# maua-maua-maua/maua

Measured on AMD Instinct MI355X. Metric: frames/sec (whole node), 1024x1024 StyleGAN2 audio-reactive render, higher is better.
Workload: dtype bf16

## Files before the change

### maua_amd/csrc/internal.h

```cpp
#pragma once
#include "common.h"

namespace maua {

int launch_pack_rgb8(hipStream_t stream, const float* img, uint8_t* out, int B, int H, int W);
template <typename TI, typename TO>
int launch_nchw_to_nhwc(hipStream_t s, const void* x, void* y, int N, int C, int HW, int Cp);
template <typename TI, typename TO>
int launch_nhwc_to_nchw(hipStream_t s, const void* x, void* y, int N, int C, int HW, int Cp);

struct ConvArgs {
  const void* x;
  long x_bstride;
  const void* w;
  const float* s;
  const float* d;
  const float* noise;
  long noise_bstride;
  float noise_strength;
  const float* noise_scale;
  const float* bias;
  void* y;
  int B, H, W, Ci, Co, up;
  int act;
// ... 60 lines not shown
  const float* noise;
  long noise_bstride;
  float noise_strength;
  const float* noise_scale;
  const float* bias;
  void* y;
  int B, H, W, Ci, Co, up, act;
  float alpha, gain, clamp;
  const float* rgb_wmod;
  const float* rgb_bias;
  const float* rgb_prev;
  float* rgb_out;
  float rgb_clamp;
  float fir[16];
  uint8_t* rgb8_out;
  int rgb_skip_f32;
};
bool hires_supported(int dtype, int Ci, int Co, int up, int H, int W);
int launch_modconv_hires(hipStream_t stream, const HiresArgs& a, int dtype = MAUA_BF16);
bool upwalk_supported(int dtype, int Ci, int Co, int up, int H, int W);
size_t upwalk_weight_elems(int Co, int Ci);
int launch_upwalk(hipStream_t stream, const HiresArgs& a, int dtype = MAUA_BF16);
int launch_prep_upwalk_weights(hipStream_t stream, const float* w, void* wt, int Co, int Ci, int flip, int dtype = MAUA_BF16);
bool upwalk_fused_supported(int dtype, int Ci, int Cm, int H, int W);
int launch_upwalk_fused(hipStream_t stream, const HiresArgs& up, const HiresArgs& c1, int force_segs = 0, int narrow_ok = 1,
                        int dtype = MAUA_BF16);

int launch_prep_weights(hipStream_t stream, int dtype, const float* w, void* wt, float* wsq, int Co, int Ci, int k,
                        int up, int flip, int Cop, int Cip);
int launch_f32_split_inplace(hipStream_t stream, void* w, long n_floats);

int launch_tconv2(hipStream_t stream, int dtype, const ConvArgs& a);
bool tconv_dma_supported(int dtype, int Ci, int Co, int H, int W);
int launch_tconv_dma(hipStream_t stream, const ConvArgs& a, int dtype = MAUA_BF16);
int launch_tconv_edges(hipStream_t stream, const ConvArgs& a, int dtype = MAUA_BF16);
int launch_prep_tconv_weights(hipStream_t stream, int dtype, const float* w, void* wt, int Co, int Ci, int flip);

struct UpfirArgs {
  const void* t;
  void* y;
  const float* d;
  const float* noise;
  long noise_bstride;
  float noise_strength;
  const float* noise_scale;
  const float* bias;
  const float* out_scale;
  int B, H, W, Co;
  int act;
  float alpha, gain, clamp;
};
int launch_upfir_epilogue(hipStream_t stream, int dtype, const UpfirArgs& a);
bool tconv_fir_supported(int dtype, int Ci, int Co, int H, int W);
int launch_tconv_fir(hipStream_t stream, const ConvArgs& a, const UpfirArgs& u, int dtype = MAUA_BF16);
size_t prepped_weight_elems(int k, int up, int Cop, int Cip);

struct LayerOperands { const void* x; const void* w; const float* s; const float* d; const float* bias; void* y; int B, H, W, Ci, Co, up; };
struct NoiseOperands { const float* noise; long bstride; float strength; const float* scale; };
struct Epilogue { int act; float alpha, gain, clamp; };
template <typename A>
inline void set_noise_args(A& a, const NoiseOperands& n) {
  a.noise = n.noise; a.noise_bstride = n.bstride; a.noise_strength = n.strength; a.noise_scale = n.scale;
}
template <typename A>
inline void set_epilogue_args(A& a, const Epilogue& e) {
  a.act = e.act; a.alpha = e.alpha; a.gain = e.gain; a.clamp = e.clamp;
}
template <typename A>
inline A layer_args(A a, const LayerOperands& l, const NoiseOperands& n, const Epilogue& e) {
  a.x = l.x; a.w = l.w; a.s = l.s; a.d = l.d; a.bias = l.bias; a.y = l.y;
  a.B = l.B; a.H = l.H; a.W = l.W; a.Ci = l.Ci; a.Co = l.Co; a.up = l.up;
  set_noise_args(a, n);
  set_epilogue_args(a, e);
  return a;
}
template <typename A>
inline void fuse_torgb_args(A& a, const float* wmod, const float* bias, const float* prev, float* out, float clamp, const float* fir16) {
  a.rgb_wmod = wmod; a.rgb_bias = bias; a.rgb_prev = prev; a.rgb_out = out; a.rgb_clamp = clamp;
  for (int i = 0; i < 16; i++) a.fir[i] = fir16[i];
}
inline void pack_u8_args(HiresArgs& a, uint8_t* rgb8_out, bool skip_f32) {
  a.rgb8_out = rgb8_out;
  a.rgb_skip_f32 = skip_f32;
}
inline ConvArgs tconv_args(const void* x, long x_bstride, const void* w, const float* s, void* t, int B, int H, int W, int Ci, int Co) {
  ConvArgs a{};
  a.x = x; a.x_bstride = x_bstride; a.w = w; a.s = s; a.y = t;
  a.B = B; a.H = H; a.W = W; a.Ci = Ci; a.Co = Co; a.up = 2;
  return a;
}
inline UpfirArgs upfir_args(void* y, const float* d, const float* bias, const float* out_scale, int B, int H, int W, int Co,
                            const NoiseOperands& n, const Epilogue& e) {
  UpfirArgs u{};
  u.y = y; u.d = d; u.bias = bias; u.out_scale = out_scale; u.B = B; u.H = H; u.W = W; u.Co = Co;
  set_noise_args(u, n);
  set_epilogue_args(u, e);
  return u;
}
inline void upsample_fir16(float* fir) {
  const float g4[4] = {0.25f, 0.75f, 0.75f, 0.25f};
  for (int u = 0; u < 4; u++)
    for (int v = 0; v < 4; v++) fir[u * 4 + v] = g4[u] * g4[v];
}

int modconv3x3_check(int dtype, const ConvArgs& a);
int lowres_check(int dtype, const ConvArgs& a);
int lowres_ksplit(int dtype, int B, int H, int W, int Ci, int Co, int up);
// ... 213 lines not shown
```

### maua_amd/csrc/modconv_api.hip

```cpp
#include <algorithm>
#include <cstring>

#include "common.h"
#include "internal.h"

namespace maua {
namespace {

enum { R_LOWRES = 0, R_GENERIC, R_DMA, R_HIRES, R_UPWALK, R_FUSED, R_WALKDONE, R_TFIR, R_TDMA, R_T2, R_UPFIR };

bool is_tconv(int r) { return r == R_TFIR || r == R_TDMA || r == R_T2; }
bool reads_premod(int r) { return r == R_TFIR || r == R_TDMA || r == R_DMA; }

LayerOperands operands(const maua_modconv_desc* d) {
  return LayerOperands{d->x, nullptr, d->s, d->d, d->bias, d->y, d->B, d->H, d->W, d->Ci, d->Co, d->up};
}
NoiseOperands noise_of(const maua_modconv_desc* d) { return NoiseOperands{d->noise, d->noise_bstride, d->noise_strength, d->noise_scale}; }
Epilogue epilogue_of(const maua_modconv_desc* d) { return Epilogue{d->act, d->alpha, d->gain, d->clamp}; }

template <typename A>
A desc_args(const maua_modconv_desc* d) {
  A a = layer_args(A{}, operands(d), noise_of(d), epilogue_of(d));
  if (d->rgb_out) {
    float fir[16];
// ... 140 lines not shown
  if (route == R_UPWALK || route == R_FUSED) {
    if (int rc = launch_prep_upwalk_weights(st, d->w, base + o_w, d->Co, d->Ci, d->flip, dtype)) return rc;
  } else if (is_tconv(route)) {
    if (int rc = launch_prep_tconv_weights(st, dtype, d->w, base + o_w, d->Co, d->Ci, d->flip)) return rc;
  } else if (route != R_UPFIR) {
    if (int rc = launch_prep_weights(st, dtype, d->w, base + o_w, nullptr, d->Co, d->Ci, 3, d->up, d->up == 2 ? d->flip : 0, d->Co, d->Ci))
      return rc;
  }
  if (route == R_FUSED)
    if (int rc = launch_prep_weights(st, dtype, d1->w, base + o_w1, nullptr, d1->Co, d1->Ci, 3, 1, 0, d1->Co, d1->Ci)) return rc;
  const void* x = d->x;
  long x_bstride = d->x_bstride;
  if (reads_premod(route)) {
    if (int rc = launch_premod_nhwc(st, d->x, d->x_bstride, d->s, base + o_xm, d->B, (long)d->H * d->W, d->Ci, dtype)) return rc;
    x = base + o_xm;
    x_bstride = (long)d->H * d->W * d->Ci;
  }
  if (ones_bytes) {
    const long n = (long)d->B * d->Ci;
    hipLaunchKernelGGL(modconv_fill_ones_kernel, dim3((unsigned)((n + 255) / 256)), dim3(256), 0, st, (float*)(base + o_ones), n);
    MAUA_HIP_CHECK(hipGetLastError());
  }
  switch (route) {
    case R_LOWRES:
    case R_GENERIC:
    case R_DMA: {
      ConvArgs a = conv_args(d);
      a.x = x; a.x_bstride = x_bstride; a.w = base + o_w;
      if (route == R_DMA) a.s = nullptr;
      return route == R_LOWRES    ? launch_modconv_lowres(st, dtype, a, base + o_xm, (float*)(base + o_ws))
             : route == R_GENERIC ? launch_modconv3x3(st, dtype, a)
                                  : launch_modconv_dma(st, a, dtype);
    }
    case R_HIRES:
    case R_UPWALK:
    case R_FUSED: {
      HiresArgs a = hires_args(d);
      a.w = base + o_w;
      if (route == R_HIRES) return launch_modconv_hires(st, a, dtype);
      if (route == R_UPWALK) return launch_upwalk(st, a, dtype);
      HiresArgs f = hires_args(d1);
      f.x = nullptr; f.y = nullptr; f.w = base + o_w1;
      a.y = nullptr;
      return launch_upwalk_fused(st, a, f, force_segs, narrow_ok, dtype);
    }
    case R_TFIR:
    case R_TDMA:
    case R_T2: {
      void* t = d->t ? d->t : base + o_t;
      ConvArgs a = tconv_args(d);
      a.x = x; a.x_bstride = x_bstride; a.w = base + o_w; a.y = t;
      if (route != R_T2) a.s = (const float*)(base + o_ones);
      UpfirArgs u = upfir_args(d);
      if (route == R_TFIR) return launch_tconv_fir(st, a, u, dtype);
      if (route == R_TDMA) {
        if (int rc = launch_tconv_edges(st, a, dtype)) return rc;
        if (int rc = launch_tconv_dma(st, a, dtype)) return rc;
      } else if (int rc = launch_tconv2(st, dtype, a)) {
        return rc;
      }
      u.t = t;
      return launch_upfir_epilogue(st, dtype, u);
    }
    case R_UPFIR: {
      UpfirArgs u = upfir_args(d);
      u.t = d->x;
      return launch_upfir_epilogue(st, dtype, u);
    }
  }
  return MAUA_OK;
}

extern "C" int maua_torgb_ex(maua_ctx* ctx, const void* x, const float* wmod, const float* bias, const float* prev, float* out, int B,
                             int H, int W, int C, float clamp, int dtype) {
  MAUA_REQUIRE(ctx && x && wmod && bias && out, "maua_torgb_ex: NULL argument");
  MAUA_REQUIRE(B >= 0 && H > 0 && W > 0 && C > 0, "maua_torgb_ex: bad shape");
  MAUA_REQUIRE(!prev || (H % 2 == 0 && W % 2 == 0), "maua_torgb_ex: the skip image needs an even grid");
  RgbArgs r{};
  r.x = x; r.wmod = wmod; r.bias = bias; r.prev = prev; r.out = out; r.B = B; r.H = H; r.W = W; r.C = C; r.clamp = clamp;
  upsample_fir16(r.fir);
  return launch_torgb(ctx->stream, dtype, r);
}
```

### maua_amd/csrc/modconv_tconv_fir.hip

```cpp
#include "common.h"
#include "internal.h"

namespace maua {

namespace {

constexpr int PTW = 32;
constexpr int HW1 = PTW + 1;
constexpr int KB = 64;
constexpr int WROWS = 9 * 32;
constexpr int WBUF = WROWS * KB;
constexpr int OFF_H = 2 * WBUF;
constexpr int ES = 128 * 2;

__device__ __constant__ const int kSlotF[9] = {0, 1, 1, 2, 2, 3, 3, 3, 3};
__device__ __constant__ const int kClsF[9] = {0, 0, 1, 0, 2, 0, 1, 2, 3};

__device__ __forceinline__ unsigned lds_off(const void* p) {
  return (unsigned)(size_t)(__attribute__((address_space(3))) const void*)p;
}
__device__ __forceinline__ void dma16_s(const void* sbase, unsigned voff, unsigned lds_dst) {
  asm volatile("s_mov_b32 m0, %2\n\ts_nop 0\n\tglobal_load_lds_dwordx4 %0, %1" ::"v"(voff), "s"(sbase), "s"(lds_dst)
               : "memory");
}
template <typename F>
__device__ __forceinline__ void mma(f32x16& acc, const u32x4& w, const u32x4& x) {
  Mma16<F>::step(acc, w, x);
}
__device__ __forceinline__ int swz(int n) { return (n >> 2) & 3; }

__device__ __forceinline__ int t_col(int tc, int pc) {
  const int p = tc >> 1;
  return p * ES + ((((tc & 1) ^ (p & 3)) << 6) | ((pc ^ ((p >> 2) & 3)) << 4));
}

template <typename F>
__device__ __forceinline__ void fir_hrow(const char* tile, int tr, const int (&tcol)[5], f32x2_t (&h)[2][4]) {
  f32x2_t c[5][4];
  const int rowb = (tr >> 1) * (PTW * ES), rsw = (tr & 1) << 7;
#pragma unroll
  for (int rx = 0; rx < 5; rx++) {
    const u32x4 v = *reinterpret_cast<const u32x4*>(tile + rowb + (tcol[rx] ^ rsw));
#pragma unroll
    for (int k = 0; k < 4; k++) c[rx][k] = f32x2_t{Fmt16<F>::lo(v[k]), Fmt16<F>::hi(v[k])};
  }
#pragma unroll
  for (int e = 0; e < 4; e++) {
    h[0][e] = (c[0][e] + c[3][e]) + 3.f * (c[1][e] + c[2][e]);
    h[1][e] = (c[1][e] + c[4][e]) + 3.f * (c[2][e] + c[3][e]);
  }
}

}

template <int PTH_, typename F>
__global__ __launch_bounds__(PTH_ * 32, PTH_ == 8 ? 2 : 1) void tconv_fir_kernel(ConvArgs a, UpfirArgs u) {
  constexpr int PTH = PTH_, UPR = PTH - 2;
  constexpr int HPX = (PTH + 1) * HW1, HBUF = HPX * KB;
  constexpr int NW = PTH / 2, NT = NW * 64;
  constexpr int WJ = (WBUF / 1024 + NW - 1) / NW, HJ = (HPX * 4 + NT - 1) / NT;
  constexpr int FG = NT / 128, FROWS = 2 * UPR / FG;
  static_assert(FG * FROWS == 2 * UPR, "output rows must split evenly over the FIR groups");
  extern __shared__ __attribute__((aligned(1024))) char smem[];
  const unsigned lds0 = __builtin_amdgcn_readfirstlane(lds_off(smem));
  const int tid = threadIdx.x, lane = tid & 63;
  const int wave = __builtin_amdgcn_readfirstlane(tid >> 6);
  const int r = lane & 31, h = lane >> 5;
  const int tiles_x = (a.W + 29) / 30, tiles = tiles_x * ((a.H + UPR - 1) / UPR), CB = a.Co >> 5;
  const int cbg = CB < 8 ? CB : 8, n_ts = tiles * a.B, per_group = ((n_ts + 7) >> 3) * 8 * cbg;
  const int L = blockIdx.x, grp = L / per_group, Lg = L - grp * per_group;
  const int xcd = Lg & 7, idx = Lg >> 3;
  const int cb = grp * cbg + idx % cbg, ts = (idx / cbg) * 8 + xcd;
  if (ts >= n_ts) return;
  const int b = ts / tiles, tile = ts - b * tiles;
  const int tyi = tile / tiles_x, txi = tile - tyi * tiles_x;
  const int ty0 = tyi * UPR - 1, tx0 = txi * 30 - 1;
  const char* xb = reinterpret_cast<const char*>(a.x) + (long)b * a.x_bstride * 2;
  const char* wp = reinterpret_cast<const char*>(a.w);

  unsigned hoff[HJ];
#pragma unroll
  for (int j = 0; j < HJ; j++) {
    const int P = (wave + NW * j) * 64 + lane;
    const int hp = P >> 2, q = (P & 3) ^ swz(hp);
    const int py = (hp * 1986) >> 16;
    const int px = hp - py * HW1;
    const int gy = ty0 - 1 + py, gx = tx0 - 1 + px;
    hoff[j] = 0xffffffffu;
    if (P < HPX * 4) {
      if (gy >= 0 && gx >= 0 && gy < a.H && gx < a.W) {
        hoff[j] = (unsigned)(((gy * a.W + gx) * a.Ci + q * 8) * 2);
      } else {
        *reinterpret_cast<u32x4*>(smem + OFF_H + P * 16) = u32x4{0u, 0u, 0u, 0u};
        *reinterpret_cast<u32x4*>(smem + OFF_H + HBUF + P * 16) = u32x4{0u, 0u, 0u, 0u};
      }
    }
  }
  unsigned woff[WJ];
#pragma unroll
  for (int j = 0; j < WJ; j++) {
    const int ii = wave + NW * j;
    const int R = min(16 * ii + (lane >> 2), WROWS - 1);
    const int k = R >> 5, n = R & 31;
    const int q = (lane & 3) ^ swz(R);
    woff[j] = (unsigned)((((((kSlotF[k] * CB + cb) * 4 + kClsF[k]) * 32 + n) * a.Ci) + q * 8) * 2);
  }
#define TD_ISSUE(C_, BUF_)                                                                               \
  {                                                                                                      \
    const char* ws_ = wp + (long)(C_) * KB;                                                              \
    _Pragma("unroll") for (int j = 0; j < WJ; j++)                                                      \
      if (wave + NW * j < WBUF / 1024) dma16_s(ws_, woff[j], lds0 + (BUF_) * WBUF + (wave + NW * j) * 1024); \
    const char* xs_ = xb + (long)(C_) * KB;                                                              \
    _Pragma("unroll") for (int j = 0; j < HJ; j++)                                                      \
      if (hoff[j] != 0xffffffffu) dma16_s(xs_, hoff[j], lds0 + OFF_H + (BUF_) * HBUF + (wave + NW * j) * 1024); \
  }

  const int hp00 = (2 * wave) * HW1 + r;
  const unsigned b0 = (unsigned)(r * KB + ((swz(r) ^ h) << 4));
#define TD_A(HR_, Q1_, KS_, BUF_)                                                                        \
  ({                                                                                                     \
    const int hp_ = hpv + (HR_) * HW1 + (Q1_);                                                           \
    *reinterpret_cast<const u32x4*>(smem + ((OFF_H + (BUF_) * HBUF + hp_ * KB + ((swz(hp_) ^ h) << 4)) ^ ((KS_) << 5))); \
  })
#define TD_B(K_, KS_, BUF_) (*reinterpret_cast<const u32x4*>(smem + (BUF_) * WBUF + (K_) * 32 * KB + (b0 ^ ((KS_) << 5))))

  f32x16 acc[2][4];
#pragma unroll
  for (int R = 0; R < 2; R++)
#pragma unroll
    for (int c = 0; c < 4; c++)
#pragma unroll
      for (int e = 0; e < 16; e++) acc[R][c][e] = 0.f;

  const int n_chunks = a.Ci >> 5;
  TD_ISSUE(0, 0)
  if (n_chunks > 1) TD_ISSUE(1, 1)
  asm volatile("s_waitcnt vmcnt(0)" ::: "memory");
  __syncthreads();
  int hpv = hp00;
#define TD_STEP(KS_, BUF_)                                                                               \
  {                                                                                                      \
    u32x4 A00 = TD_A(0, 0, KS_, BUF_), A01 = TD_A(0, 1, KS_, BUF_);      \
    u32x4 A10 = TD_A(1, 0, KS_, BUF_), A11 = TD_A(1, 1, KS_, BUF_);                    \
    u32x4 A20 = TD_A(2, 0, KS_, BUF_), A21 = TD_A(2, 1, KS_, BUF_);                    \
    {                                                                                                    \
      const u32x4 B0 = TD_B(0, KS_, BUF_), B1 = TD_B(1, KS_, BUF_), B2 = TD_B(2, KS_, BUF_);              \
      mma<F>(acc[0][0], B0, A00); mma<F>(acc[1][0], B0, A10);                                 \
      mma<F>(acc[0][1], B2, A01); mma<F>(acc[1][1], B2, A11);                        \
      mma<F>(acc[0][0], B1, A01); mma<F>(acc[1][0], B1, A11);                        \
    }                                                                                                    \
    {                                                                                                    \
      const u32x4 B3 = TD_B(3, KS_, BUF_), B4 = TD_B(4, KS_, BUF_);                                       \
      mma<F>(acc[0][2], B4, A10); mma<F>(acc[1][2], B4, A20);                        \
      mma<F>(acc[0][0], B3, A10); mma<F>(acc[1][0], B3, A20);                        \
    }                                                                                                    \
    {                                                                                                    \
      const u32x4 B5 = TD_B(5, KS_, BUF_), B6 = TD_B(6, KS_, BUF_), B7 = TD_B(7, KS_, BUF_), B8 = TD_B(8, KS_, BUF_); \
      mma<F>(acc[0][3], B8, A11); mma<F>(acc[1][3], B8, A21);                                 \
      mma<F>(acc[0][1], B6, A11); mma<F>(acc[1][1], B6, A21);                                                  \
      mma<F>(acc[0][2], B7, A11); mma<F>(acc[1][2], B7, A21);                                                  \
      mma<F>(acc[0][0], B5, A11); mma<F>(acc[1][0], B5, A21);                                                  \
    }                                                                                                    \
  }
  for (int c = 0; c < n_chunks; c++) {
    const int buf = c & 1;
    asm volatile("" : "+v"(hpv));
    TD_STEP(0, buf)
    {
      u32x4 A00 = TD_A(0, 0, 1, buf), A01 = TD_A(0, 1, 1, buf), A10 = TD_A(1, 0, 1, buf), A11 = TD_A(1, 1, 1, buf);
      u32x4 A20 = TD_A(2, 0, 1, buf), A21 = TD_A(2, 1, 1, buf);
      const u32x4 B0 = TD_B(0, 1, buf), B1 = TD_B(1, 1, buf), B2 = TD_B(2, 1, buf), B3 = TD_B(3, 1, buf), B4 = TD_B(4, 1, buf);
      const u32x4 B5 = TD_B(5, 1, buf), B6 = TD_B(6, 1, buf), B7 = TD_B(7, 1, buf), B8 = TD_B(8, 1, buf);
      asm volatile("s_waitcnt vmcnt(0)" ::: "memory");
      __syncthreads();
      if (c + 2 < n_chunks) TD_ISSUE(c + 2, buf)
      mma<F>(acc[0][0], B0, A00); mma<F>(acc[1][0], B0, A10);
      mma<F>(acc[0][1], B2, A01); mma<F>(acc[1][1], B2, A11);
      mma<F>(acc[0][0], B1, A01); mma<F>(acc[1][0], B1, A11);
      mma<F>(acc[0][2], B4, A10); mma<F>(acc[1][2], B4, A20);
      mma<F>(acc[0][0], B3, A10); mma<F>(acc[1][0], B3, A20);
      mma<F>(acc[0][3], B8, A11); mma<F>(acc[1][3], B8, A21);
      mma<F>(acc[0][1], B6, A11); mma<F>(acc[1][1], B6, A21);
      mma<F>(acc[0][2], B7, A11); mma<F>(acc[1][2], B7, A21);
      mma<F>(acc[0][0], B5, A11); mma<F>(acc[1][0], B5, A21);
    }
  }
#undef TD_ISSUE
#undef TD_A
#undef TD_B
#undef TD_STEP

  const int fhalf = tid / 120, fw = tid - fhalf * 120;
  const int strip = fw >> 2, pc = fw & 3;
  const int xl = 2 + 2 * strip, yl0 = 2 + FROWS * fhalf;
  const int X = 2 * tx0 + xl, Wo = 2 * a.W, Ho = 2 * a.H;
  const int cho = cb * 32 + pc * 8;
  const bool fir_on = tid < 120 * FG && X < Wo;
  f32x2_t dv[4], bv[4], sv[4];
  float2 nzv[FROWS];
#pragma unroll
  for (int k = 0; k < FROWS; k++) nzv[k] = make_float2(0.f, 0.f);
  if (fir_on) {
#pragma unroll
    for (int e4 = 0; e4 < 8; e4 += 4) {
      const float4 s4 = u.out_scale ? *reinterpret_cast<const float4*>(u.out_scale + (long)b * a.Co + cho + e4)
                                    : make_float4(1.f, 1.f, 1.f, 1.f);
      sv[e4 / 2] = f32x2_t{s4.x, s4.y}; sv[e4 / 2 + 1] = f32x2_t{s4.z, s4.w};
      const float4 d4 = u.d ? *reinterpret_cast<const float4*>(u.d + (long)b * a.Co + cho + e4) : make_float4(1.f, 1.f, 1.f, 1.f);
      const float4 b4 = u.bias ? *reinterpret_cast<const float4*>(u.bias + cho + e4) : make_float4(0.f, 0.f, 0.f, 0.f);
      dv[e4 / 2] = f32x2_t{d4.x, d4.y}; dv[e4 / 2 + 1] = f32x2_t{d4.z, d4.w};
      bv[e4 / 2] = f32x2_t{b4.x, b4.y}; bv[e4 / 2 + 1] = f32x2_t{b4.z, b4.w};
    }
    if (u.noise) {
      const float* nb = u.noise + (long)b * u.noise_bstride;
#pragma unroll
      for (int k = 0; k < FROWS; k++) {
        const int Y = 2 * ty0 + yl0 + k;
        if (Y < Ho) nzv[k] = *reinterpret_cast<const float2*>(nb + (long)Y * Wo + X);
      }
    }
  }
  __syncthreads();
  char* tt = smem;
#pragma unroll
  for (int R = 0; R < 2; R++) {
    const int m = (2 * wave + R) * 32 + r;
#pragma unroll
    for (int c = 0; c < 4; c++)
#pragma unroll
      for (int qd = 0; qd < 4; qd++)
        *reinterpret_cast<uint2*>(tt + m * ES + (((c ^ (r & 3)) << 6) | ((qd ^ ((r >> 2) & 3)) << 4) | (h << 3))) =
            make_uint2(Fmt16<F>::pack2(acc[R][c][qd * 4 + 0], acc[R][c][qd * 4 + 1]), Fmt16<F>::pack2(acc[R][c][qd * 4 + 2], acc[R][c][qd * 4 + 3]));
  }
  __syncthreads();
  {
    if (fir_on) {
#pragma unroll
      for (int e = 0; e < 4; e++) { dv[e] *= 0.0625f * u.gain; bv[e] *= u.gain; }
      const float nzs = u.noise_strength * u.gain * (u.noise_scale ? u.noise_scale[b] : 1.f);
      const float cl = u.clamp >= 0.f ? u.clamp : 3.0e38f;
      char* yb = reinterpret_cast<char*>(u.y) + (long)b * Ho * Wo * a.Co * 2;
      int tcol[5];
#pragma unroll
      for (int rx = 0; rx < 5; rx++) tcol[rx] = t_col(xl - 1 + rx, pc);
      f32x2_t hr[4][2][4];
      fir_hrow<F>(tt, yl0 - 1, tcol, hr[0]);
      fir_hrow<F>(tt, yl0, tcol, hr[1]);
      fir_hrow<F>(tt, yl0 + 1, tcol, hr[2]);
#pragma unroll
      for (int k = 0; k < FROWS; k++) {
        fir_hrow<F>(tt, yl0 + k + 2, tcol, hr[(k + 3) & 3]);
        const int Y = 2 * ty0 + yl0 + k;
        if (Y < Ho) {
          const float nz[2] = {nzv[k].x * nzs, nzv[k].y * nzs};
#pragma unroll
          for (int j = 0; j < 2; j++) {
            f32x2_t o[4];
#pragma unroll
            for (int e = 0; e < 4; e++) {
              const f32x2_t accv = (hr[k & 3][j][e] + hr[(k + 3) & 3][j][e]) + 3.f * (hr[(k + 1) & 3][j][e] + hr[(k + 2) & 3][j][e]);
              f32x2_t t = accv * dv[e] + (bv[e] + nz[j]);
              const f32x2_t ta = t * u.alpha;
              t = f32x2_t{fmaxf(t[0], ta[0]), fmaxf(t[1], ta[1])};
              o[e] = f32x2_t{__builtin_amdgcn_fmed3f(t[0], -cl, cl), __builtin_amdgcn_fmed3f(t[1], -cl, cl)} * sv[e];
            }
            *reinterpret_cast<u32x4*>(yb + (((long)Y * Wo + X + j) * a.Co + cho) * 2) =
                u32x4{Fmt16<F>::pack2(o[0][0], o[0][1]), Fmt16<F>::pack2(o[1][0], o[1][1]), Fmt16<F>::pack2(o[2][0], o[2][1]), Fmt16<F>::pack2(o[3][0], o[3][1])};
          }
        }
      }
    }
  }
}

bool tconv_fir_supported(int dtype, int Ci, int Co, int H, int W) {
  return (dtype == MAUA_BF16 || dtype == MAUA_F16) && Ci % 32 == 0 && Co % 32 == 0 && H >= 16 && W >= 32 && (long)H * W * Ci * 2 < (1L << 32) &&
         16L * Co * Ci * 2 < (1L << 32);
}

int tconv_fir_check(const ConvArgs& a, const UpfirArgs& u, int dtype) {
  MAUA_REQUIRE(tconv_fir_supported(dtype, a.Ci, a.Co, a.H, a.W), "tconv_fir: unsupported shape");
  MAUA_REQUIRE(u.act == MAUA_ACT_LRELU && u.alpha >= 0.f && u.alpha <= 1.f && u.gain > 0.f, "tconv_fir: lrelu epilogue only");
  MAUA_REQUIRE(!u.noise || (((uintptr_t)u.noise % 8) == 0 && u.noise_bstride % 2 == 0), "tconv_fir: noise must be 8-byte aligned");
  const int pth = 8, upr = pth - 2;
  const int tiles = ((a.H + upr - 1) / upr) * ((a.W + 29) / 30), CB = a.Co / 32, cbg = CB < 8 ? CB : 8;
  MAUA_REQUIRE(CB % cbg == 0, "tconv_fir: channel blocks must split into groups of 8");
  const long n_ts = (long)tiles * a.B, grid = ((n_ts + 7) / 8) * 8 * cbg * (CB / cbg);
  MAUA_REQUIRE(grid < (1L << 31), "tconv_fir: grid too large");
  return MAUA_OK;
}

int launch_tconv_fir(hipStream_t stream, const ConvArgs& a, const UpfirArgs& u, int dtype) {
  if (int rc = tconv_fir_check(a, u, dtype)) return rc;
  if (a.B == 0) return MAUA_OK;
  const int pth = 8, upr = pth - 2;
  const int tiles = ((a.H + upr - 1) / upr) * ((a.W + 29) / 30), CB = a.Co / 32, cbg = CB < 8 ? CB : 8;
  const long n_ts = (long)tiles * a.B, grid = ((n_ts + 7) / 8) * 8 * cbg * (CB / cbg);
  const size_t smem = std::max<size_t>((size_t)2 * WBUF + 2 * (pth + 1) * HW1 * KB, (size_t)pth * PTW * ES);
  if (dtype == MAUA_F16) {
    MAUA_HIP_CHECK(hipFuncSetAttribute((const void*)tconv_fir_kernel<8, f16_t>, hipFuncAttributeMaxDynamicSharedMemorySize, (int)smem));
    hipLaunchKernelGGL((tconv_fir_kernel<8, f16_t>), dim3((unsigned)grid), dim3(256), smem, stream, a, u);
  } else {
    MAUA_HIP_CHECK(hipFuncSetAttribute((const void*)tconv_fir_kernel<8, bf16_t>, hipFuncAttributeMaxDynamicSharedMemorySize, (int)smem));
    hipLaunchKernelGGL((tconv_fir_kernel<8, bf16_t>), dim3((unsigned)grid), dim3(256), smem, stream, a, u);
  }
  MAUA_HIP_CHECK(hipGetLastError());
  return MAUA_OK;
}

}
```

### maua_amd/csrc/synth.hip

```cpp
#include <cmath>
#include <cstring>
#include <string>
#include <vector>

#include "common.h"
#include "internal.h"

using namespace maua;

namespace {

struct ConvLayer {
  int block, which;
  int Ci, Co, res, up, w_index;
  int ih = 0, iw = 0;
  int oh = 0, ow = 0;
  int fh = 0, fw = 0;
  float* affine_w = nullptr;
  float* affine_b = nullptr;
  float* bias = nullptr;
  float* noise_const = nullptr;
  float noise_strength = 0.f;
  void* wt = nullptr;
  void* wt_t = nullptr;
  void* wt_h = nullptr;
  float* wsq = nullptr;
  float* s = nullptr;
  float* d = nullptr;
  void* feat = nullptr;
};
struct RgbLayer {
  int block, C, res, w_index;
  int h = 0, w = 0;
  float* affine_w = nullptr;
  float* affine_b = nullptr;
  float* wrgb = nullptr;
  float* bias = nullptr;
  float* s = nullptr;
  float* wmod = nullptr;
};

template <typename T>
int dev_alloc(T** p, size_t n) {
  MAUA_HIP_CHECK(hipMalloc((void**)p, n * sizeof(T)));
  return MAUA_OK;
}

}

struct maua_synth {
  maua_ctx* ctx;
  int res, w_dim, channel_base, channel_max, dtype, nv_compat;
  int nblocks, num_ws;
  size_t esize;
  std::vector<ConvLayer> convs;
  std::vector<RgbLayer> rgbs;
  void* const_x = nullptr;
  int keep_features = 0;
  int lowres = 1;
  int use_hires = 1;
  int upwalk = 2;
  int walk_segs = 0;
  int walk_narrow = 1;
  int fuse_torgb = 1;
  int tconv_up = 1;
  int tconv_fir = 256;
  const float* nz_scales = nullptr;
  long nz_scale_stride = 0;
  int dma_conv = 1;
  int dual_store = 1;
  int tconv_dma = 1;
  float* ones = nullptr;
  void* xm = nullptr;
  void* tbuf = nullptr;
  void* lowres_xm = nullptr;
  float* lowres_ws = nullptr;
  int rs_layer = -1, rs_mode = 0, rs_th = 0, rs_tw = 0, rs_pl = 0, rs_pr = 0, rs_pt = 0, rs_pb = 0, rs_how = 3;
  float rs_value = 0.f;
  float* rs_noise = nullptr;
  void* const_rs = nullptr;
  float* rgb_tmp[2] = {nullptr, nullptr};
  int out_h = 0, out_w = 0;
  int warp_layer[3] = {-1, -1, -1};
  const float* warp_minv[3] = {nullptr, nullptr, nullptr};
  int profile = 0;
  std::vector<hipEvent_t> ev;
  size_t ev_used = 0;
  std::vector<size_t> ev_fwd_start;
  int bcap = 0;
  void* act[2] = {nullptr, nullptr};
  float* img[2] = {nullptr, nullptr};
  StyleLayer* style_table_dev = nullptr;
  float fir[16];
};

static void prof_mark(maua_synth* n) {
  if (!n->profile || n->ev_used >= (1u << 16)) return;
  if (n->ev_used == n->ev.size()) {
    hipEvent_t e;
    if (hipEventCreate(&e) != hipSuccess) return;
    n->ev.push_back(e);
  }
  hipEventRecord(n->ev[n->ev_used++], n->ctx->stream);
}

static int channels_for(int res, int base, int maxc) { return std::min(base / res, maxc); }

static bool lowres_fits(const maua_synth* n, const ConvLayer& c) {
  return lowres_supported(n->dtype, c.Ci, c.Co, c.up, c.ih, c.iw);
}
static bool tconv_dma_fits(const maua_synth* n, const ConvLayer& c) {
  return c.up == 2 && tconv_dma_supported(n->dtype, c.Ci, c.Co, c.ih, c.iw);
}

static void compute_dims(maua_synth* n) {
  int h = 4, w = 4;
  if (n->rs_layer == 0) { h = n->rs_th; w = n->rs_tw; }
  size_t li = 0;
  for (int blk = 0; blk < n->nblocks; blk++) {
// ... 362 lines not shown
    MAUA_HIP_CHECK(hipMemcpy(n->rs_noise, fill_noise_host, cnt * sizeof(float), hipMemcpyHostToDevice));
  }
  compute_dims(n);
  free_workspace(n);
  for (size_t i = 0; i < n->convs.size(); i++) {
    ConvLayer& c = n->convs[i];
    if (c.oh != before[i].oh || c.ow != before[i].ow) {
      hipFree(c.noise_const);
      c.noise_const = nullptr;
      MAUA_HIP_CHECK(hipMalloc((void**)&c.noise_const, (size_t)c.oh * c.ow * sizeof(float)));
      MAUA_HIP_CHECK(hipMemset(c.noise_const, 0, (size_t)c.oh * c.ow * sizeof(float)));
    }
  }
  return MAUA_OK;
}

int maua_synth_set_warp(maua_synth* n, int slot, int layer, const float* inv_matrices_dev) {
  MAUA_REQUIRE(n, "maua_synth_set_warp: net is NULL");
  MAUA_REQUIRE(slot >= 0 && slot < 3, "maua_synth_set_warp: slot must be 0..2");
  MAUA_REQUIRE(layer >= 1 && layer <= (int)n->convs.size(), "maua_synth_set_warp: layer must name a synthesis layer (1-based index into layer_names)");
  n->warp_layer[slot] = inv_matrices_dev ? layer : -1;
  n->warp_minv[slot] = inv_matrices_dev;
  return MAUA_OK;
}

int maua_synth_layer_size(const maua_synth* n, int layer, int* h, int* w) {
  MAUA_REQUIRE(n && h && w, "maua_synth_layer_size: NULL argument");
  MAUA_REQUIRE(layer >= -1 && layer < (int)n->convs.size(), "maua_synth_layer_size: no such layer");
  if (layer < 0) { *h = n->out_h; *w = n->out_w; }
  else { *h = n->convs[layer].oh; *w = n->convs[layer].ow; }
  return MAUA_OK;
}

int maua_synth_set_option(maua_synth* n, const char* key, int value) {
  MAUA_REQUIRE(n && key, "maua_synth_set_option: NULL argument");
  if (!strcmp(key, "profile")) {
    n->profile = value;
    n->ev_used = 0;
    n->ev_fwd_start.clear();
    return MAUA_OK;
  }
  if (!strcmp(key, "keep_features")) {
    if (n->keep_features != value) {
      MAUA_HIP_CHECK(hipStreamSynchronize(n->ctx->stream));
      free_workspace(n);
      n->keep_features = value;
    }
    return MAUA_OK;
  }
  static const std::pair<const char*, int maua_synth::*> routing[] = {
      {"lowres", &maua_synth::lowres},         {"use_hires", &maua_synth::use_hires}, {"upwalk", &maua_synth::upwalk},
      {"walk_segs", &maua_synth::walk_segs},   {"walk_narrow", &maua_synth::walk_narrow},
      {"fuse_torgb", &maua_synth::fuse_torgb}, {"tconv_up", &maua_synth::tconv_up},   {"tconv_fir", &maua_synth::tconv_fir},
      {"tconv_dma", &maua_synth::tconv_dma},   {"dma_conv", &maua_synth::dma_conv},   {"dual_store", &maua_synth::dual_store}};
  for (const auto& o : routing)
    if (!strcmp(key, o.first)) {
      n->*o.second = value;
      return MAUA_OK;
    }
  return fail(std::string("maua_synth_set_option: unknown option ") + key);
}

static thread_local hipMemcpyKind g_load_kind = hipMemcpyHostToDevice;

static int upload(float* dst, const float* host, size_t count, size_t expect, const char* name) {
  if (count != expect)
    return fail(std::string("maua_synth_load: ") + name + ": expected " + std::to_string(expect) + " values, got " +
                std::to_string(count));
  MAUA_HIP_CHECK(hipMemcpy(dst, host, count * sizeof(float), g_load_kind));
  return MAUA_OK;
}

int maua_synth_load(maua_synth* n, const char* name, const float* host, size_t count) {
  MAUA_REQUIRE(n && name && host, "maua_synth_load: NULL argument");
  std::string s(name);
  int blk = -1, pos = 0;
  if (sscanf(name, "bs.%d.%n", &blk, &pos) < 1 || blk < 0 || blk >= n->nblocks || pos == 0)
    return fail("maua_synth_load: unknown parameter name: " + s);
  std::string rest = s.substr(pos);
  hipStream_t st = n->ctx->stream;
  auto check_filter = [&]() -> int {
    if (count != 16) return fail("maua_synth_load: " + s + ": only the 4x4 [1,3,3,1] resample filter is supported");
    const float t[4] = {1, 3, 3, 1};
    for (int u = 0; u < 4; u++)
      for (int v = 0; v < 4; v++)
        if (std::fabs(host[u * 4 + v] - t[u] * t[v] / 64.f) > 1e-6f)
          return fail("maua_synth_load: " + s + ": only the 4x4 [1,3,3,1] resample filter is supported");
    return MAUA_OK;
  };
  if (rest == "resample_filter") return check_filter();
  if (rest == "const") {
    if (blk != 0) return fail("maua_synth_load: only block 0 has a const input");
    int C = n->convs[0].Ci;
    if (count != (size_t)C * 16) return fail("maua_synth_load: bs.0.const: wrong size");
    float* tmp;
    MAUA_HIP_CHECK(hipMalloc((void**)&tmp, count * 4));
    MAUA_HIP_CHECK(hipMemcpy(tmp, host, count * 4, g_load_kind));
    int rc = n->dtype == MAUA_BF16   ? launch_nchw_to_nhwc<float, bf16_t>(st, tmp, n->const_x, 1, C, 16, C)
             : n->dtype == MAUA_F16 ? launch_nchw_to_nhwc<float, f16_t>(st, tmp, n->const_x, 1, C, 16, C)
                                    : launch_nchw_to_nhwc<float, float>(st, tmp, n->const_x, 1, C, 16, C);
    hipStreamSynchronize(st);
    hipFree(tmp);
    return rc;
  }
  size_t dot = rest.find('.');
  if (dot == std::string::npos) return fail("maua_synth_load: unknown parameter name: " + s);
// ... 115 lines not shown
      const ConvLayer& c = n->convs[li];
      const Step& s = plan.conv[li];
      const bool hooked = n->rs_layer == (int)li + 1;
      void* y = n->keep_features && !hooked ? c.feat : n->act[cur];
      const float* next_s = s.scale_next ? n->convs[li + 1].s : nullptr;
      switch (s.route) {
        case Route::Lowres:
        case Route::Generic:
        case Route::DmaConv1: {
          ConvArgs a = layer_args(ConvArgs{}, li, x, y);
          a.x_bstride = x_bstride;
          a.out_scale = next_s;
          if (s.dual) a.y_scaled = n->xm;
          if (s.rgb) fuse_torgb(a);
          if (s.route == Route::DmaConv1) a.s = nullptr;
          if (int rc = s.route == Route::Lowres    ? launch_modconv_lowres(st, n->dtype, a, n->lowres_xm, n->lowres_ws)
                       : s.route == Route::Generic ? launch_modconv3x3(st, n->dtype, a)
                                                   : launch_modconv_dma(st, a, n->dtype))
            return rc;
          break;
        }
        case Route::Hires:
        case Route::Upwalk:
        case Route::FusedWalk: {
          HiresArgs a = layer_args(HiresArgs{}, li, x, s.skip_store ? nullptr : y);
          if (s.rgb) fuse_torgb(a);
          if (s.rgb8) pack_u8(a);
          if (s.route != Route::Hires) a.w = c.wt_h;
          if (s.route != Route::FusedWalk) {
            if (int rc = s.route == Route::Hires ? launch_modconv_hires(st, a, n->dtype) : launch_upwalk(st, a, n->dtype)) return rc;
            break;
          }
          HiresArgs f = layer_args(HiresArgs{}, li + 1, nullptr, nullptr);
          fuse_torgb(f);
          if (plan.conv[li + 1].rgb8) pack_u8(f);
          if (int rc = launch_upwalk_fused(st, a, f, n->walk_segs, n->walk_narrow, n->dtype)) return rc;
          break;
        }
        case Route::WalkDone:
          break;
        case Route::TconvFir:
        case Route::TconvDma:
        case Route::Tconv2: {
          ConvArgs a = tconv_args(x, x_bstride, c.wt_t, c.s, n->tbuf, B, c.ih, c.iw, c.Ci, c.Co);
          UpfirArgs u = upfir_args(y, c.d, c.bias, next_s, B, c.ih, c.iw, c.Co, layer_noise(li), lrelu_epilogue());
          if (s.src == Src::PremodPass)
            if (int rc = launch_premod_nhwc(st, x, x_bstride, c.s, n->xm, B, (long)c.ih * c.iw, c.Ci, n->dtype)) return rc;
          if (s.src == Src::PremodPass || s.src == Src::Xm) {
            a.x = n->xm;
            a.x_bstride = (long)c.ih * c.iw * c.Ci;
          }
          if (reads_premod(s.route)) a.s = n->ones;
          if (s.route == Route::TconvFir) {
            if (int rc = launch_tconv_fir(st, a, u, n->dtype)) return rc;
            prof_mark(n);
            break;
          }
          if (s.route == Route::TconvDma) {
            if (int rc = launch_tconv_edges(st, a, n->dtype)) return rc;
            if (int rc = launch_tconv_dma(st, a, n->dtype)) return rc;
          } else if (int rc = launch_tconv2(st, n->dtype, a)) {
            return rc;
          }
          prof_mark(n);
          u.t = n->tbuf;
          if (int rc = launch_upfir_epilogue(st, n->dtype, u)) return rc;
          break;
        }
      }
      prof_mark(n);
      x = y;
      x_bstride = (long)c.oh * c.ow * c.Co;
      cur ^= 1;
      if (hooked) {
        void* dst = n->keep_features ? c.feat : n->act[cur];
        if (int rc = resize_feat(x, x_bstride, B, c.oh, c.ow, c.Co, dst)) return rc;
        x = dst;
        x_bstride = (long)c.fh * c.fw * c.Co;
        cur ^= 1;
      }
      for (int wsl = 0; wsl < 3; wsl++) {
        if (n->warp_layer[wsl] != (int)li + 1 || !n->warp_minv[wsl]) continue;
        void* dst = n->act[cur];
        if (dst == x) dst = n->act[cur ^ 1];
        if (int rc = launch_warp_affine_nhwc(st, n->dtype, x, dst, n->warp_minv[wsl], B, c.fh, c.fw, c.Co)) return rc;
        if (n->keep_features) {
          MAUA_HIP_CHECK(hipMemcpyAsync(c.feat, dst, (size_t)B * c.fh * c.fw * c.Co * n->esize, hipMemcpyDeviceToDevice, st));
        } else {
          x = dst;
          cur = (dst == n->act[0]) ? 1 : 0;
        }
      }
    }
    if (plan.rgb[blk] != RgbRoute::Fused) {
      const bool hook = plan.rgb[blk] == RgbRoute::Hook;
      RgbArgs r{};
      r.x = x; r.wmod = g.wmod; r.bias = g.bias; r.prev = hook ? nullptr : prev_img;
      r.out = hook ? n->rgb_tmp[0] : rgb_out; r.B = B; r.H = g.h; r.W = g.w; r.C = g.C; r.clamp = 256.f;
      memcpy(r.fir, n->fir, sizeof(r.fir));
      if (int rc = launch_torgb(st, n->dtype, r)) return rc;
      if (hook) {
        const ConvLayer& hc = n->convs[n->rs_layer - 1];
        const int nh = hc.oh, nw = hc.ow;
        ResizeArgs inv{};
        inv.x = n->rgb_tmp[0]; inv.x_bstride = 3L * g.h * g.w; inv.y = n->rgb_tmp[1]; inv.B = B; inv.H = g.h; inv.W = g.w;
        inv.C = 3; inv.oh = nh; inv.ow = nw; inv.mode = n->rs_mode; inv.pl = -n->rs_pl; inv.pt = -n->rs_pt;
        inv.how = MAUA_PAD_CONSTANT; inv.value = 0.f; inv.noise = nullptr;
// ... 91 lines not shown
```

Measured before the change: 4589.

## Walk tconv+FIR tiles vertically, carrying halo t rows between steps

Adds a walking variant of the fused transposed-conv + FIR kernel. Each block now steps down a column segment in 8-row steps and carries the last three t rows in registers/LDS, so the overlapping halo rows are no longer recomputed as they are with independent 6-row tiles. A host-side planner chooses the segment count from the CU count to balance occupancy against walk length, and the mode is on by default. The cost is longer-running blocks with a sequential dependency, extra LDS, and fewer blocks available for parallelism.

```diff
diff --git a/maua_amd/csrc/internal.h b/maua_amd/csrc/internal.h
--- a/maua_amd/csrc/internal.h
+++ b/maua_amd/csrc/internal.h
@@ -136,7 +136,7 @@
 };
 int launch_upfir_epilogue(hipStream_t stream, int dtype, const UpfirArgs& a);
 bool tconv_fir_supported(int dtype, int Ci, int Co, int H, int W);
-int launch_tconv_fir(hipStream_t stream, const ConvArgs& a, const UpfirArgs& u, int dtype = MAUA_BF16);
+int launch_tconv_fir(hipStream_t stream, const ConvArgs& a, const UpfirArgs& u, int dtype = MAUA_BF16, int walk = 1, int force_segs = 0);
 size_t prepped_weight_elems(int k, int up, int Cop, int Cip);
 
 struct LayerOperands { const void* x; const void* w; const float* s; const float* d; const float* bias; void* y; int B, H, W, Ci, Co, up; };
diff --git a/maua_amd/csrc/modconv_api.hip b/maua_amd/csrc/modconv_api.hip
--- a/maua_amd/csrc/modconv_api.hip
+++ b/maua_amd/csrc/modconv_api.hip
@@ -216,7 +216,7 @@
       a.x = x; a.x_bstride = x_bstride; a.w = base + o_w; a.y = t;
       if (route != R_T2) a.s = (const float*)(base + o_ones);
       UpfirArgs u = upfir_args(d);
-      if (route == R_TFIR) return launch_tconv_fir(st, a, u, dtype);
+      if (route == R_TFIR) return launch_tconv_fir(st, a, u, dtype, force_segs >= 0, force_segs);
       if (route == R_TDMA) {
         if (int rc = launch_tconv_edges(st, a, dtype)) return rc;
         if (int rc = launch_tconv_dma(st, a, dtype)) return rc;
diff --git a/maua_amd/csrc/modconv_tconv_fir.hip b/maua_amd/csrc/modconv_tconv_fir.hip
--- a/maua_amd/csrc/modconv_tconv_fir.hip
+++ b/maua_amd/csrc/modconv_tconv_fir.hip
@@ -53,20 +53,22 @@
 
 }
 
-template <int PTH_, typename F>
-__global__ __launch_bounds__(PTH_ * 32, PTH_ == 8 ? 2 : 1) void tconv_fir_kernel(ConvArgs a, UpfirArgs u) {
+template <int PTH_, typename F, bool WALK>
+__global__ __launch_bounds__(PTH_ * 32, PTH_ == 8 ? 2 : 1) void tconv_fir_kernel(ConvArgs a, UpfirArgs u, int nseg, int seg_steps) {
   constexpr int PTH = PTH_, UPR = PTH - 2;
+  static_assert(!WALK || PTH_ == 8, "the walk carries three t rows of a 16-row tile");
   constexpr int HPX = (PTH + 1) * HW1, HBUF = HPX * KB;
   constexpr int NW = PTH / 2, NT = NW * 64;
   constexpr int WJ = (WBUF / 1024 + NW - 1) / NW, HJ = (HPX * 4 + NT - 1) / NT;
-  constexpr int FG = NT / 128, FROWS = 2 * UPR / FG;
-  static_assert(FG * FROWS == 2 * UPR, "output rows must split evenly over the FIR groups");
+  constexpr int FG = NT / 128, FROWS = (WALK ? 2 * PTH : 2 * UPR) / FG;
+  static_assert(FG * FROWS == (WALK ? 2 * PTH : 2 * UPR), "output rows must split evenly over the FIR groups");
+  constexpr int OFF_T = WALK ? 2 * PTW * ES : 0;
   extern __shared__ __attribute__((aligned(1024))) char smem[];
   const unsigned lds0 = __builtin_amdgcn_readfirstlane(lds_off(smem));
   const int tid = threadIdx.x, lane = tid & 63;
   const int wave = __builtin_amdgcn_readfirstlane(tid >> 6);
   const int r = lane & 31, h = lane >> 5;
-  const int tiles_x = (a.W + 29) / 30, tiles = tiles_x * ((a.H + UPR - 1) / UPR), CB = a.Co >> 5;
+  const int tiles_x = (a.W + 29) / 30, tiles = tiles_x * (WALK ? nseg : (a.H + UPR - 1) / UPR), CB = a.Co >> 5;
   const int cbg = CB < 8 ? CB : 8, n_ts = tiles * a.B, per_group = ((n_ts + 7) >> 3) * 8 * cbg;
   const int L = blockIdx.x, grp = L / per_group, Lg = L - grp * per_group;
   const int xcd = Lg & 7, idx = Lg >> 3;
@@ -74,14 +76,56 @@
   if (ts >= n_ts) return;
   const int b = ts / tiles, tile = ts - b * tiles;
   const int tyi = tile / tiles_x, txi = tile - tyi * tiles_x;
-  const int ty0 = tyi * UPR - 1, tx0 = txi * 30 - 1;
+  const int tx0 = txi * 30 - 1;
+  int step = 0, step_end = 1, y_lo = 0, y_hi = 2 * a.H;
+  if (WALK) {
+    const int n_steps = (a.H >> 3) + 1, s0 = tyi ? seg_steps + (tyi - 1) * (seg_steps - 1) : 0;
+    step_end = min(n_steps, tyi ? s0 + seg_steps - 1 : seg_steps);
+    step = tyi ? s0 - 1 : 0;
+    y_lo = tyi ? 16 * s0 - 2 : 0;
+    if (step_end < n_steps) y_hi = 16 * step_end - 2;
+  }
   const char* xb = reinterpret_cast<const char*>(a.x) + (long)b * a.x_bstride * 2;
   const char* wp = reinterpret_cast<const char*>(a.w);
 
+  unsigned woff[WJ];
+#pragma unroll
+  for (int j = 0; j < WJ; j++) {
+    const int ii = wave + NW * j;
+    const int R = min(16 * ii + (lane >> 2), WROWS - 1);
+    const int k = R >> 5, n = R & 31;
+    const int q = (lane & 3) ^ swz(R);
+    woff[j] = (unsigned)((((((kSlotF[k] * CB + cb) * 4 + kClsF[k]) * 32 + n) * a.Ci) + q * 8) * 2);
+  }
+#define TD_ISSUE(C_, BUF_)                                                                               \
+  {                                                                                                      \
+    const char* ws_ = wp + (long)(C_) * KB;                                                              \
+    _Pragma("unroll") for (int j = 0; j < WJ; j++)                                                      \
+      if (wave + NW * j < WBUF / 1024) dma16_s(ws_, woff[j], lds0 + (BUF_) * WBUF + (wave + NW * j) * 1024); \
+    const char* xs_ = xb + (long)(C_) * KB;                                                              \
+    _Pragma("unroll") for (int j = 0; j < HJ; j++)                                                      \
+      if (hoff[j] != 0xffffffffu) dma16_s(xs_, hoff[j], lds0 + OFF_H + (BUF_) * HBUF + (wave + NW * j) * 1024); \
+  }
+
+  const int hp00 = (2 * wave) * HW1 + r;
+  const unsigned b0 = (unsigned)(r * KB + ((swz(r) ^ h) << 4));
+#define TD_A(HR_, Q1_, KS_, BUF_)                                                                        \
+  ({                                                                                                     \
+    const int hp_ = hpv + (HR_) * HW1 + (Q1_);                                                           \
+    *reinterpret_cast<const u32x4*>(smem + ((OFF_H + (BUF_) * HBUF + hp_ * KB + ((swz(hp_) ^ h) << 4)) ^ ((KS_) << 5))); \
+  })
+#define TD_B(K_, KS_, BUF_) (*reinterpret_cast<const u32x4*>(smem + (BUF_) * WBUF + (K_) * 32 * KB + (b0 ^ ((KS_) << 5))))
+
+  u32x4 carry[3] = {u32x4{0u, 0u, 0u, 0u}, u32x4{0u, 0u, 0u, 0u}, u32x4{0u, 0u, 0u, 0u}};
+  const int n_chunks = a.Ci >> 5;
+  do {
+  int tidh = tid;
+  if (WALK) asm volatile("" : "+v"(tidh));
+  const int ty0 = WALK ? 8 * step : tyi * UPR - 1;
   unsigned hoff[HJ];
 #pragma unroll
   for (int j = 0; j < HJ; j++) {
-    const int P = (wave + NW * j) * 64 + lane;
+    const int P = (wave + NW * j) * 64 + (tidh & 63);
     const int hp = P >> 2, q = (P & 3) ^ swz(hp);
     const int py = (hp * 1986) >> 16;
     const int px = hp - py * HW1;
@@ -96,34 +140,6 @@
       }
     }
   }
-  unsigned woff[WJ];
-#pragma unroll
-  for (int j = 0; j < WJ; j++) {
-    const int ii = wave + NW * j;
-    const int R = min(16 * ii + (lane >> 2), WROWS - 1);
-    const int k = R >> 5, n = R & 31;
-    const int q = (lane & 3) ^ swz(R);
-    woff[j] = (unsigned)((((((kSlotF[k] * CB + cb) * 4 + kClsF[k]) * 32 + n) * a.Ci) + q * 8) * 2);
-  }
-#define TD_ISSUE(C_, BUF_)                                                                               \
-  {                                                                                                      \
-    const char* ws_ = wp + (long)(C_) * KB;                                                              \
-    _Pragma("unroll") for (int j = 0; j < WJ; j++)                                                      \
-      if (wave + NW * j < WBUF / 1024) dma16_s(ws_, woff[j], lds0 + (BUF_) * WBUF + (wave + NW * j) * 1024); \
-    const char* xs_ = xb + (long)(C_) * KB;                                                              \
-    _Pragma("unroll") for (int j = 0; j < HJ; j++)                                                      \
-      if (hoff[j] != 0xffffffffu) dma16_s(xs_, hoff[j], lds0 + OFF_H + (BUF_) * HBUF + (wave + NW * j) * 1024); \
-  }
-
-  const int hp00 = (2 * wave) * HW1 + r;
-  const unsigned b0 = (unsigned)(r * KB + ((swz(r) ^ h) << 4));
-#define TD_A(HR_, Q1_, KS_, BUF_)                                                                        \
-  ({                                                                                                     \
-    const int hp_ = hpv + (HR_) * HW1 + (Q1_);                                                           \
-    *reinterpret_cast<const u32x4*>(smem + ((OFF_H + (BUF_) * HBUF + hp_ * KB + ((swz(hp_) ^ h) << 4)) ^ ((KS_) << 5))); \
-  })
-#define TD_B(K_, KS_, BUF_) (*reinterpret_cast<const u32x4*>(smem + (BUF_) * WBUF + (K_) * 32 * KB + (b0 ^ ((KS_) << 5))))
-
   f32x16 acc[2][4];
 #pragma unroll
   for (int R = 0; R < 2; R++)
@@ -132,7 +148,6 @@
 #pragma unroll
       for (int e = 0; e < 16; e++) acc[R][c][e] = 0.f;
 
-  const int n_chunks = a.Ci >> 5;
   TD_ISSUE(0, 0)
   if (n_chunks > 1) TD_ISSUE(1, 1)
   asm volatile("s_waitcnt vmcnt(0)" ::: "memory");
@@ -185,22 +200,16 @@
       mma<F>(acc[0][0], B5, A11); mma<F>(acc[1][0], B5, A21);
     }
   }
-#undef TD_ISSUE
-#undef TD_A
-#undef TD_B
-#undef TD_STEP
-
-  const int fhalf = tid / 120, fw = tid - fhalf * 120;
+  int tidf = tid;
+  if (WALK) asm volatile("" : "+v"(tidf));
+  const int fhalf = tidf / 120, fw = tidf - fhalf * 120;
   const int strip = fw >> 2, pc = fw & 3;
-  const int xl = 2 + 2 * strip, yl0 = 2 + FROWS * fhalf;
-  const int X = 2 * tx0 + xl, Wo = 2 * a.W, Ho = 2 * a.H;
+  const int xl = 2 + 2 * strip, yl0 = (WALK ? -2 : 2) + FROWS * fhalf;
+  const int X = 2 * tx0 + xl, Wo = 2 * a.W;
   const int cho = cb * 32 + pc * 8;
-  const bool fir_on = tid < 120 * FG && X < Wo;
+  const bool fir_on = tidf < 120 * FG && X < Wo;
   f32x2_t dv[4], bv[4], sv[4];
-  float2 nzv[FROWS];
-#pragma unroll
-  for (int k = 0; k < FROWS; k++) nzv[k] = make_float2(0.f, 0.f);
-  if (fir_on) {
+  auto load_channel_vectors = [&]() {
 #pragma unroll
     for (int e4 = 0; e4 < 8; e4 += 4) {
       const float4 s4 = u.out_scale ? *reinterpret_cast<const float4*>(u.out_scale + (long)b * a.Co + cho + e4)
@@ -211,35 +220,49 @@
       dv[e4 / 2] = f32x2_t{d4.x, d4.y}; dv[e4 / 2 + 1] = f32x2_t{d4.z, d4.w};
       bv[e4 / 2] = f32x2_t{b4.x, b4.y}; bv[e4 / 2 + 1] = f32x2_t{b4.z, b4.w};
     }
+  };
+  const int coff2 = (tidf >> 3) * ES + (((tidf >> 3) & 2) ? 0 : 128) + (tidf & 7) * 16;
+  const bool fir_step = !WALK || 16 * step + 14 > y_lo;
+  float2 nzv[FROWS];
+#pragma unroll
+  for (int k = 0; k < FROWS; k++) nzv[k] = make_float2(0.f, 0.f);
+  if (fir_on && fir_step) {
+    load_channel_vectors();
     if (u.noise) {
       const float* nb = u.noise + (long)b * u.noise_bstride;
 #pragma unroll
       for (int k = 0; k < FROWS; k++) {
         const int Y = 2 * ty0 + yl0 + k;
-        if (Y < Ho) nzv[k] = *reinterpret_cast<const float2*>(nb + (long)Y * Wo + X);
+        if (Y >= y_lo && Y < y_hi) nzv[k] = *reinterpret_cast<const float2*>(nb + (long)Y * Wo + X);
       }
     }
   }
   __syncthreads();
-  char* tt = smem;
+  char* tt = smem + OFF_T;
+  const int rt = tidf & 31, ht = (tidf >> 5) & 1;
 #pragma unroll
   for (int R = 0; R < 2; R++) {
-    const int m = (2 * wave + R) * 32 + r;
+    const int m = (2 * wave + R) * 32 + rt;
 #pragma unroll
     for (int c = 0; c < 4; c++)
 #pragma unroll
       for (int qd = 0; qd < 4; qd++)
-        *reinterpret_cast<uint2*>(tt + m * ES + (((c ^ (r & 3)) << 6) | ((qd ^ ((r >> 2) & 3)) << 4) | (h << 3))) =
+        *reinterpret_cast<uint2*>(tt + m * ES + (((c ^ (rt & 3)) << 6) | ((qd ^ ((rt >> 2) & 3)) << 4) | (ht << 3))) =
             make_uint2(Fmt16<F>::pack2(acc[R][c][qd * 4 + 0], acc[R][c][qd * 4 + 1]), Fmt16<F>::pack2(acc[R][c][qd * 4 + 2], acc[R][c][qd * 4 + 3]));
+  }
+  if (WALK) {
+    *reinterpret_cast<u32x4*>(smem + PTW * ES + tidf * 16) = carry[0];
+    *reinterpret_cast<u32x4*>(smem + PTW * ES + 4096 + tidf * 16) = carry[1];
+    *reinterpret_cast<u32x4*>(smem + coff2) = carry[2];
   }
   __syncthreads();
   {
-    if (fir_on) {
+    if (fir_on && fir_step) {
 #pragma unroll
       for (int e = 0; e < 4; e++) { dv[e] *= 0.0625f * u.gain; bv[e] *= u.gain; }
       const float nzs = u.noise_strength * u.gain * (u.noise_scale ? u.noise_scale[b] : 1.f);
       const float cl = u.clamp >= 0.f ? u.clamp : 3.0e38f;
-      char* yb = reinterpret_cast<char*>(u.y) + (long)b * Ho * Wo * a.Co * 2;
+      char* yb = reinterpret_cast<char*>(u.y) + (long)b * (2 * a.H) * Wo * a.Co * 2;
       int tcol[5];
 #pragma unroll
       for (int rx = 0; rx < 5; rx++) tcol[rx] = t_col(xl - 1 + rx, pc);
@@ -251,7 +274,7 @@
       for (int k = 0; k < FROWS; k++) {
         fir_hrow<F>(tt, yl0 + k + 2, tcol, hr[(k + 3) & 3]);
         const int Y = 2 * ty0 + yl0 + k;
-        if (Y < Ho) {
+        if (Y >= y_lo && Y < y_hi) {
           const float nz[2] = {nzv[k].x * nzs, nzv[k].y * nzs};
 #pragma unroll
           for (int j = 0; j < 2; j++) {
@@ -271,6 +294,16 @@
       }
     }
   }
+  if (!WALK || ++step >= step_end) break;
+  carry[0] = *reinterpret_cast<const u32x4*>(tt + 7 * PTW * ES + tidf * 16);
+  carry[1] = *reinterpret_cast<const u32x4*>(tt + 7 * PTW * ES + 4096 + tidf * 16);
+  carry[2] = *reinterpret_cast<const u32x4*>(tt + 6 * PTW * ES + coff2);
+  __syncthreads();
+  } while (true);
+#undef TD_ISSUE
+#undef TD_A
+#undef TD_B
+#undef TD_STEP
 }
 
 bool tconv_fir_supported(int dtype, int Ci, int Co, int H, int W) {
@@ -290,20 +323,39 @@
   return MAUA_OK;
 }
 
-int launch_tconv_fir(hipStream_t stream, const ConvArgs& a, const UpfirArgs& u, int dtype) {
+static void tconv_walk_plan(const ConvArgs& a, int slots, int force_segs, int* nseg, int* seg_steps) {
+  const int n_steps = a.H / 8 + 1, max_segs = std::max(1, n_steps / 2);
+  const long per_seg = (long)a.B * (a.Co / 32) * ((a.W + 29) / 30);
+  long best = -1;
+  for (int cand = 1; cand <= max_segs; cand++) {
+    if (force_segs > 0 && cand != std::min(force_segs, max_segs)) continue;
+    const int steps = (n_steps + cand - 1 + cand - 1) / cand;
+    const int segs = n_steps > steps ? 1 + (n_steps - steps + steps - 2) / (steps - 1) : 1;
+    const long cost = ((per_seg * segs + slots - 1) / slots) * steps;
+    if (best < 0 || cost < best) { best = cost; *nseg = segs; *seg_steps = steps; }
+  }
+}
+
+int launch_tconv_fir(hipStream_t stream, const ConvArgs& a, const UpfirArgs& u, int dtype, int walk, int force_segs) {
   if (int rc = tconv_fir_check(a, u, dtype)) return rc;
   if (a.B == 0) return MAUA_OK;
   const int pth = 8, upr = pth - 2;
-  const int tiles = ((a.H + upr - 1) / upr) * ((a.W + 29) / 30), CB = a.Co / 32, cbg = CB < 8 ? CB : 8;
+  const int CB = a.Co / 32, cbg = CB < 8 ? CB : 8;
+  int nseg = 1, seg_steps = 1;
+  if (walk) {
+    int dev = 0, cus = 256;
+    MAUA_HIP_CHECK(hipGetDevice(&dev));
+    MAUA_HIP_CHECK(hipDeviceGetAttribute(&cus, hipDeviceAttributeMultiprocessorCount, dev));
+    tconv_walk_plan(a, 2 * cus, force_segs, &nseg, &seg_steps);
+  }
+  const int tiles = (walk ? nseg : (a.H + upr - 1) / upr) * ((a.W + 29) / 30);
   const long n_ts = (long)tiles * a.B, grid = ((n_ts + 7) / 8) * 8 * cbg * (CB / cbg);
-  const size_t smem = std::max<size_t>((size_t)2 * WBUF + 2 * (pth + 1) * HW1 * KB, (size_t)pth * PTW * ES);
-  if (dtype == MAUA_F16) {
-    MAUA_HIP_CHECK(hipFuncSetAttribute((const void*)tconv_fir_kernel<8, f16_t>, hipFuncAttributeMaxDynamicSharedMemorySize, (int)smem));
-    hipLaunchKernelGGL((tconv_fir_kernel<8, f16_t>), dim3((unsigned)grid), dim3(256), smem, stream, a, u);
-  } else {
-    MAUA_HIP_CHECK(hipFuncSetAttribute((const void*)tconv_fir_kernel<8, bf16_t>, hipFuncAttributeMaxDynamicSharedMemorySize, (int)smem));
-    hipLaunchKernelGGL((tconv_fir_kernel<8, bf16_t>), dim3((unsigned)grid), dim3(256), smem, stream, a, u);
-  }
+  const size_t kbuf = (size_t)2 * WBUF + 2 * (pth + 1) * HW1 * KB;
+  const size_t smem = std::max<size_t>(kbuf, (size_t)(pth + (walk ? 2 : 0)) * PTW * ES);
+  auto kern = dtype == MAUA_F16 ? (walk ? tconv_fir_kernel<8, f16_t, true> : tconv_fir_kernel<8, f16_t, false>)
+                                : (walk ? tconv_fir_kernel<8, bf16_t, true> : tconv_fir_kernel<8, bf16_t, false>);
+  MAUA_HIP_CHECK(hipFuncSetAttribute((const void*)kern, hipFuncAttributeMaxDynamicSharedMemorySize, (int)smem));
+  hipLaunchKernelGGL(kern, dim3((unsigned)grid), dim3(256), smem, stream, a, u, nseg, seg_steps);
   MAUA_HIP_CHECK(hipGetLastError());
   return MAUA_OK;
 }
diff --git a/maua_amd/csrc/synth.hip b/maua_amd/csrc/synth.hip
--- a/maua_amd/csrc/synth.hip
+++ b/maua_amd/csrc/synth.hip
@@ -65,6 +65,7 @@
   int fuse_torgb = 1;
   int tconv_up = 1;
   int tconv_fir = 256;
+  int tconv_walk = 1;
   const float* nz_scales = nullptr;
   long nz_scale_stride = 0;
   int dma_conv = 1;
@@ -533,6 +534,7 @@
       {"lowres", &maua_synth::lowres},         {"use_hires", &maua_synth::use_hires}, {"upwalk", &maua_synth::upwalk},
       {"walk_segs", &maua_synth::walk_segs},   {"walk_narrow", &maua_synth::walk_narrow},
       {"fuse_torgb", &maua_synth::fuse_torgb}, {"tconv_up", &maua_synth::tconv_up},   {"tconv_fir", &maua_synth::tconv_fir},
+      {"tconv_walk", &maua_synth::tconv_walk},
       {"tconv_dma", &maua_synth::tconv_dma},   {"dma_conv", &maua_synth::dma_conv},   {"dual_store", &maua_synth::dual_store}};
   for (const auto& o : routing)
     if (!strcmp(key, o.first)) {
@@ -754,7 +756,7 @@
           }
           if (reads_premod(s.route)) a.s = n->ones;
           if (s.route == Route::TconvFir) {
-            if (int rc = launch_tconv_fir(st, a, u, n->dtype)) return rc;
+            if (int rc = launch_tconv_fir(st, a, u, n->dtype, n->tconv_walk, 0)) return rc;
             prof_mark(n);
             break;
           }
```

Result: faster. 4640, median of 6 (+1.1%).
